# BerserkerMother/Video-Summarization

Measured on AMD Instinct MI355X. Metric: frames/sec scored (whole node), synthetic [B,T=1024,D=1024], higher is better.
Workload: dtype f32; 1 GPU; configs[2]: B=64 videos x T=1024 frames x D=1024 per GPU, scorer cfg M-A (heads 4, d_model 256, layers 4), logits + hidden state; global_batch=64, parallelism=videos sharded over 1 GPU(s), no all_gather of scores

## Files before the change

### video-summarization_amd/csrc/vs_attention.hip

```cpp
#include "vs_device.h"
#include "vs_kernels.h"

namespace {

template <int DH, int NKB, bool VARLEN = false>
__global__ __launch_bounds__(256, 2) void attn_fwd(
    const float *__restrict__ Q, const float *__restrict__ Kg, const float *__restrict__ Vg,
    const uint8_t *__restrict__ mask, float *__restrict__ out, int H, int T, float scale_log2e, int BH,
    const int *__restrict__ cu = nullptr, const int2 *__restrict__ work = nullptr, int Mtot = 0) {
    constexpr int KT = 32 * NKB, LD = DH + 4, NJ = DH / 8, ND = DH / 32;
    constexpr int F4 = KT * DH / 4 / 256;
    __shared__ __attribute__((aligned(16))) float Ks[KT * LD];
    __shared__ __attribute__((aligned(16))) float Vs[KT * LD];
    __shared__ float mb[KT];

    const int tid = threadIdx.x, lane = tid & 63, wave = tid >> 6;
    const int r = lane & 31, h = lane >> 5;
    int b, head, qt;
    size_t base, orow0;
    if constexpr (VARLEN) {
        const int2 wk = work[blockIdx.x];
        b = wk.x; qt = wk.y; head = blockIdx.y;
        const int c0 = cu[b];
        T = cu[b + 1] - c0;
// ... 744 lines not shown
    };
    if constexpr (DMA) {
#pragma unroll
        for (int u = 0; u < KAHEAD; ++u) dma_issue(u, u, true, u < VAHEAD);
#pragma unroll
        for (int u = 0; u < KAHEAD; ++u) { gload_m(u); stage_m(u % NMB); }
        gload_m(KAHEAD);
        asm volatile("s_waitcnt vmcnt(0)" ::: "memory");
    } else {
#pragma unroll
        for (int u = 0; u < KAHEAD; ++u) {
            gload_k(u); gload_m(u);
            if (u < VAHEAD) gload_v(u);
#pragma unroll
            for (int i = 0; i < KPT; ++i) stage_k1(i, u % NBUF);
            if (u < VAHEAD) {
#pragma unroll
                for (int e = 0; e < 4; ++e) stage_v1(e, u % NBUF);
            }
            stage_m(u % NMB);
        }
        gload_k(KAHEAD); gload_m(KAHEAD); gload_v(VAHEAD);
    }
    __syncthreads();
    f32x16 sa[2], sb[2];
#pragma unroll
    for (int n = 0; n < 2; ++n)
#pragma unroll
        for (int t = 0; t < 16; ++t) { sa[n][t] = 0.f; sb[n][t] = 0.f; }
#pragma unroll
    for (int ks = 0; ks < NS; ++ks)
#pragma unroll
        for (int n = 0; n < 2; ++n) {
            u32x4 ka[NP];
            k_frag(0, ks, n, ka);
            static_for<NPROD>([&](auto prc) { mma_prod(prc, ka, qreg[ks], sa[n]); });
        }

    constexpr float CMARGIN = PREC == 2 ? -8.0f : 6.0f;
    (void)CMARGIN;
    u32x4 pf[2][2][NP];
    f16x2 pmaxh = {(_Float16)0.f, (_Float16)0.f};
    float cb_a = 0.f, cb_b = 0.f;
    auto rebase = [&](f32x16 (&sv)[2], float &cb, bool raise) __attribute__((always_inline)) {
        float mx = __builtin_fmaxf(__builtin_fmaxf(sv[0][0], sv[0][1]), sv[1][0]);
        mx = __builtin_fmaxf(mx, sv[1][1]);
#pragma unroll
        for (int t = 2; t < 16; t += 2) {
            mx = __builtin_fmaxf(__builtin_fmaxf(mx, sv[0][t]), sv[0][t + 1]);
            mx = __builtin_fmaxf(__builtin_fmaxf(mx, sv[1][t]), sv[1][t + 1]);
        }
        const float raw = pair_max(mx) + cb;
        float c_new = m_run;
        if ((raise || m_run == NEG_INF) && raw + CMARGIN > m_run) {
            const float cl = __builtin_fminf(__builtin_fmaxf(raw + CMARGIN, -32768.f), 32768.f);
            const unsigned b = __builtin_bit_cast(unsigned, cl);
            constexpr unsigned LOW = PREC == 2 ? 0x1FFFu : 0xFFFFu;
            c_new = __builtin_bit_cast(float, (cl >= 0.f ? b + LOW : b) & ~LOW);
            if (PREC == 1 && __builtin_fabsf(cl) >= 8192.f) c_new = __builtin_bit_cast(float, (b + 0x8000u) & ~LOW);
            if (PREC == 2 && __builtin_fabsf(c_new) < 0.0001220703125f) c_new = cl > 0.f ? 0.0001220703125f : 0.f;
        }
        const float u_new = (c_new == NEG_INF) ? 0.f : c_new;
        const float shift = cb - u_new;
        const float alpha = __builtin_amdgcn_exp2f(m_run - u_new);
#pragma unroll
        for (int n = 0; n < 2; ++n)
#pragma unroll
            for (int t = 0; t < 16; ++t) sv[n][t] += shift;
#pragma unroll
        for (int d = 0; d <= ND; ++d)
#pragma unroll
            for (int t = 0; t < 16; ++t) o[d][t] *= alpha;
        m_run = c_new;
        cb = u_new;
        unsigned pl[NP];
        pack(-u_new, 0.f, pl);
        nbias = h == 0 ? pl[0] : 0u;
    };
    auto p_pair = [&](auto kc, f32x16 (&sv)[2]) __attribute__((always_inline)) {
        constexpr int k = decltype(kc)::value, n = k / 8, ks = (k / 4) % 2, j = k % 4;
        unsigned pl[NP];
        pack(__builtin_amdgcn_exp2f(sv[n][8 * ks + 2 * j]), __builtin_amdgcn_exp2f(sv[n][8 * ks + 2 * j + 1]), pl);
#pragma unroll
        for (int p = 0; p < NP; ++p) pf[n][ks][p][j] = pl[p];
        if constexpr (PREC == 2) pmaxh = __builtin_elementwise_max(pmaxh, __builtin_bit_cast(f16x2, pl[0]));
    };
    float sm_mx = 0.f;
    f32x2 sm_mm = {0.f, 0.f};
    auto sm_unit_max = [&](auto uc, f32x16 (&sv)[2]) __attribute__((always_inline)) {
        constexpr int U = decltype(uc)::value;
        constexpr float THR = 8.0f;
        if constexpr (U == 0) {
            sm_mx = __builtin_fmaxf(__builtin_fmaxf(sv[0][0], sv[0][1]), sv[1][0]);
            sm_mx = __builtin_fmaxf(sm_mx, sv[1][1]);
        }
        if constexpr (U < 4) {
            constexpr int t0 = U == 0 ? 2 : 4 * U;
#pragma unroll
            for (int t = t0; t < 4 * U + 4; t += 2) {
                sm_mx = __builtin_fmaxf(__builtin_fmaxf(sm_mx, sv[0][t]), sv[0][t + 1]);
                sm_mx = __builtin_fmaxf(__builtin_fmaxf(sm_mx, sv[1][t]), sv[1][t + 1]);
            }
        }
        if constexpr (U == 4) {
            const float mx = pair_max(sm_mx);
            const bool raise = mx > m_run + THR || (m_run == NEG_INF && mx != NEG_INF);
            if (__builtin_expect(__any(raise), 0)) {
                const float m_new = raise ? mx : m_run;
                const float u_new = (m_new == NEG_INF) ? 0.f : m_new;
                const float alpha = __builtin_amdgcn_exp2f(m_run - u_new);
#pragma unroll
                for (int d = 0; d <= ND; ++d)
#pragma unroll
                    for (int t = 0; t < 16; ++t) o[d][t] *= alpha;
                m_run = m_new;
            }
            const float m_use = (m_run == NEG_INF) ? 0.f : m_run;
            sm_mm[0] = m_use; sm_mm[1] = m_use;
        }
        if constexpr (U >= 5 && U < 21) {
            constexpr int k = U - 5, n = k / 8, ks = (k / 4) % 2, j = k % 4;
            const f32x2 sx = {sv[n][8 * ks + 2 * j], sv[n][8 * ks + 2 * j + 1]};
            const f32x2 dv = sx - sm_mm;
            unsigned pl[NP];
            pack(__builtin_amdgcn_exp2f(dv[0]), __builtin_amdgcn_exp2f(dv[1]), pl);
#pragma unroll
            for (int p = 0; p < NP; ++p) pf[n][ks][p][j] = pl[p];
        }
    };
    auto sm_unit = [&](auto uc, f32x16 (&sv)[2], float &cb) __attribute__((always_inline)) {
        constexpr int U = decltype(uc)::value;
        if constexpr (!FOLD) { sm_unit_max(uc, sv); return; }
        if constexpr (U == 0) {
            const float u_run = (m_run == NEG_INF) ? 0.f : m_run;
            if (__builtin_expect(__any(cb != u_run || m_run == NEG_INF), 0)) rebase(sv, cb, false);
        }
        if constexpr (U >= 1 && U < 17) p_pair(std::integral_constant<int, U - 1>{}, sv);
        if constexpr (U == 17) {
            unsigned acc = 0u;
            bool hit;
            if constexpr (PREC == 2) {
                acc = __builtin_bit_cast(unsigned, pmaxh);
                hit = (acc & 0xFFFFu) >= 0x7800u || (acc >> 16) >= 0x7800u;
                pmaxh = f16x2{(_Float16)0.f, (_Float16)0.f};
            } else {
#pragma unroll
                for (int n = 0; n < 2; ++n)
#pragma unroll
                    for (int ks = 0; ks < 2; ++ks) acc |= (pf[n][ks][0][0] | pf[n][ks][0][1]) | (pf[n][ks][0][2] | pf[n][ks][0][3]);
                hit = (acc & 0x40004000u) != 0u;
            }
            if (__builtin_expect(__any(hit), 0)) {
                const unsigned hbit = hit ? 1u : 0u;
                auto pr = __builtin_amdgcn_permlane32_swap(hbit, hbit, false, false);
                rebase(sv, cb, (((unsigned)pr[0] | (unsigned)pr[1]) & 1u) != 0u);
                static_for<16>([&](auto kc) { p_pair(kc, sv); });
                if constexpr (PREC == 2) pmaxh = f16x2{(_Float16)0.f, (_Float16)0.f};
            }
        }
    };
    constexpr int NU = FOLD ? 18 : 21;
    constexpr bool FULLPF = PREC == 1 && DH <= 64;
    constexpr int NKF = FULLPF ? NS * 2 : 2, NVF = FULLPF ? 4 * ND : 2;
    constexpr int NBIAS = FOLD ? 2 : 0;
    constexpr int NSLOT_A = 2 * NS * NPROD + NBIAS, RA = (NU + NSLOT_A - 1) / NSLOT_A;
    constexpr int NSLOT_B = 4 * (ND * NPROD + NP);
    constexpr int NITEM = KPT + 4 + 2, SB = NSLOT_B / NITEM > 0 ? NSLOT_B / NITEM : 1;

    u32x4 abl_frag = {0u, 0u, 0u, 0u};
    if constexpr ((ABL & 16) != 0) abl_frag = *(const u32x4 *)&Kb[0][0][r * LDK + 8 * h];
    auto iteration = [&](int t, f32x16 (&s_in)[2], float &cb_in, f32x16 (&s_out)[2], float &cb_out) __attribute__((always_inline)) {
        const int cur = (ABL & 4) ? 0 : t % NBUF, nxt = (ABL & 4) ? 0 : (t + 1) % NBUF;
        if (mask != nullptr || (t + 1) * KT > T) {
            const float *mp = mb[t % NMB];
#pragma unroll
            for (int n = 0; n < 2; ++n)
#pragma unroll
                for (int g = 0; g < 4; ++g) {
                    const f32x4 bv = *(const f32x4 *)&mp[32 * n + 8 * g + 4 * h];
#pragma unroll
                    for (int e = 0; e < 4; ++e) s_in[n][4 * g + e] += bv[e];
                }
        }
        cb_out = (m_run == NEG_INF) ? 0.f : m_run;
        const u32x4 nb = {nbias, 0u, 0u, 0u};
        const f32x16 zero16 = {0.f, 0.f, 0.f, 0.f, 0.f, 0.f, 0.f, 0.f, 0.f, 0.f, 0.f, 0.f, 0.f, 0.f, 0.f, 0.f};
        u32x4 ka[NKF][NP], va[NVF][NP];
        if constexpr ((ABL & 16) != 0) {
#pragma unroll
            for (int g = 0; g < NKF; ++g)
#pragma unroll
                for (int p = 0; p < NP; ++p) ka[g][p] = abl_frag;
#pragma unroll
            for (int g = 0; g < NVF; ++g)
#pragma unroll
                for (int p = 0; p < NP; ++p) va[g][p] = abl_frag;
        } else
        if constexpr (FULLPF) {
#pragma unroll
            for (int g = 0; g < NS * 2; ++g) k_frag(nxt, g % NS, g / NS, ka[g]);
        } else {
            k_frag(nxt, 0, 0, ka[0]);
        }
        __builtin_amdgcn_sched_barrier(0);
        static_for<NSLOT_A>([&](auto ic) {
            constexpr int i = decltype(ic)::value, PERN = NS * NPROD, n = i < NBIAS ? i : (i - NBIAS) / PERN,
                          w = i < NBIAS ? 0 : 1 + (i - NBIAS) % PERN;
            if constexpr (w == 0) {
                s_out[n] = mma(ones_u, nb, zero16);
            } else {
                constexpr int ks = (w - 1) / NPROD, pr = (w - 1) % NPROD, g = n * NS + ks;
                if constexpr (!FOLD && w == 1) s_out[n] = zero16;
                if constexpr (!(ABL & 16) && !FULLPF && pr == 0 && g + 1 < NS * 2) k_frag(nxt, (g + 1) % NS, (g + 1) / NS, ka[(g + 1) & 1]);
                mma_prod(std::integral_constant<int, pr>{}, ka[FULLPF ? g : (g & 1)], qreg[ks], s_out[n]);
            }
            if constexpr (!(ABL & 16) && FULLPF && i >= NBIAS && i - NBIAS < NVF) {
                constexpr int f = i - NBIAS;
                v_frag(cur, f / ND / 2, (f / ND) % 2, f % ND, va[f]);
            }
            static_for<RA>([&](auto rc) {
                constexpr int U = i * RA + decltype(rc)::value;
                if constexpr (U < NU && !(ABL & 8)) sm_unit(std::integral_constant<int, U>{}, s_in, cb_in);
            });
            __builtin_amdgcn_sched_barrier(0);
        });
        lap(1);
        if constexpr (DMA) asm volatile("s_waitcnt vmcnt(0)" ::: "memory");
        if constexpr (STAG && !(ABL & 2)) { __syncthreads(); lap(3); }
        if constexpr (!FULLPF && !(ABL & 16)) v_frag(cur, 0, 0, 0, va[0]);
        __builtin_amdgcn_sched_barrier(0);
        static_for<NSLOT_B>([&](auto ic) {
            constexpr int i = decltype(ic)::value;
            constexpr int PER = ND * NPROD + NP;
            constexpr int g = i / PER, w = i % PER, n = g / 2, ks = g % 2;
            if constexpr (w < ND * NPROD) {
                constexpr int d = w / NPROD, pr = w % NPROD, f = g * ND + d;
                if constexpr (!(ABL & 16) && !FULLPF && pr == 0 && f + 1 < 4 * ND)
                    v_frag(cur, (f + 1) / ND / 2, ((f + 1) / ND) % 2, (f + 1) % ND, va[(f + 1) & 1]);
                mma_prod(std::integral_constant<int, pr>{}, va[FULLPF ? f : (f & 1)], pf[n][ks], o[d]);
            } else {
                constexpr int p = NP - 1 - (w - ND * NPROD);
                o[ND] = mma(ones_u, pf[n][ks][p], o[ND]);
            }
            if constexpr (DMA) {
                if constexpr (!(ABL & 1) && i == 0) dma_issue(t + KAHEAD, t + VAHEAD, true, true);
                if constexpr (!(ABL & 1) && i == 4) { stage_m((t + KAHEAD) % NMB); gload_m(t + KAHEAD + 1); }
            } else
            if constexpr (!(ABL & 1) && i % SB == SB - 1 && i / SB < NITEM) {
                constexpr int item = i / SB;
                if constexpr (item < KPT) stage_k1(item, (t + KAHEAD) % NBUF);
                else if constexpr (item < KPT + 4) stage_v1(item - KPT, (t + VAHEAD) % NBUF);
                else if constexpr (item == KPT + 4) { stage_m((t + KAHEAD) % NMB); }
                else { gload_k(t + KAHEAD + 1); gload_m(t + KAHEAD + 1); gload_v(t + VAHEAD + 1); }
            }
            __builtin_amdgcn_sched_barrier(0);
        });
        lap(2);
        if constexpr (!(ABL & 2)) __syncthreads();
        lap(3);
    };

    lap(0);
    const bool late = STAG && __builtin_amdgcn_readfirstlane(wave) >= NW / 2;
    if (late) __syncthreads();
    int t = 0;
    for (; t + 1 < ntiles; t += 2) {
        iteration(t, sa, cb_a, sb, cb_b);
        iteration(t + 1, sb, cb_b, sa, cb_a);
    }
    if (t < ntiles) iteration(t, sa, cb_a, sb, cb_b);
    if (STAG && !late) __syncthreads();

    const int q = q0 + r;
    if (q < T) {
        const float inv = 1.0f / o[ND][0];
        float *op = out + (orow0 + q) * (H * DH) + head * DH;
        h16 *op16 = (h16 *)out + (orow0 + q) * (H * DH) + head * DH;
#pragma unroll
        for (int d = 0; d < ND; ++d)
#pragma unroll
            for (int g = 0; g < 4; ++g) {
                f32x4 v;
#pragma unroll
                for (int e = 0; e < 4; ++e) v[e] = o[d][4 * g + e] * inv;
                if constexpr (IO16) {
                    u32x2 u; u[0] = pack_bf16(v[0], v[1]); u[1] = pack_bf16(v[2], v[3]);
                    *(u32x2 *)(op16 + 32 * d + 8 * g + 4 * h) = u;
                } else
                *(f32x4 *)(op + 32 * d + 8 * g + 4 * h) = v;
            }
    }
    if constexpr (DIAG != 0) {
        asm volatile("s_waitcnt vmcnt(0)" ::: "memory");
        lap(7);
        dg[8] = tl - tbeg; dg[10] = __builtin_amdgcn_s_memrealtime(); dg[11] = (unsigned long long)ntiles;
        if (diag != nullptr && lane == 0) {
            unsigned long long *o_ = diag + ((size_t)blockIdx.x * NW + wave) * 16;
#pragma unroll
            for (int i = 0; i < 12; ++i) o_[i] = dg[i];
        }
    }
}

template <int DH, bool HAS_MASK, int NW, bool VARLEN = false, int DIAG = 0>
__global__ __launch_bounds__(64 * NW, 2) void attn_fwd_pipe(
    const float *__restrict__ Q, const float *__restrict__ Kg, const float *__restrict__ Vg,
    const uint8_t *__restrict__ mask, float *__restrict__ out, int H, int T, float scale_log2e, int BH,
    const int *__restrict__ cu = nullptr, const int2 *__restrict__ work = nullptr, int Mtot = 0,
    unsigned long long *__restrict__ diag = nullptr) {
    unsigned long long dg[13] = {0ull, 0ull, 0ull, 0ull, 0ull, 0ull, 0ull, 0ull, 0ull, 0ull, 0ull, 0ull, 0ull}, tbeg = 0, tl = 0;
    if constexpr (DIAG != 0) { dg[9] = __builtin_amdgcn_s_memrealtime(); tbeg = vs_stamp(); tl = tbeg; }
    auto lap = [&](int slot) __attribute__((always_inline)) {
        if constexpr (DIAG != 0) { const unsigned long long t = vs_stamp(); dg[slot] += t - tl; tl = t; }
    };
    constexpr int KT = 64, LD = DH + 4, NJ = DH / 8, ND = DH / 32;
    constexpr int NT = 64 * NW;
    constexpr int F4 = KT * DH / 4 / NT;
    constexpr int TILE = KT * LD;
    constexpr float THR = 8.0f;
    __shared__ __attribute__((aligned(16))) float smem[4 * TILE + 2 * KT];
    float *mbs = smem + 4 * TILE;

    const int tid = threadIdx.x, lane = tid & 63, wave = tid >> 6;
    const int r = lane & 31, h = lane >> 5;
    int b, head, qt;
    size_t base, orow0;
    if constexpr (VARLEN) {
        const int2 wk = work[blockIdx.x];
        b = wk.x; qt = wk.y; head = blockIdx.y;
        const int c0 = cu[b];
        T = cu[b + 1] - c0;
        base = ((size_t)head * Mtot + c0) * DH;
        orow0 = (size_t)c0;
    } else {
        int bh;
        if (!attn_block_map((T + 32 * NW - 1) / (32 * NW), BH, bh, qt)) return;
        b = bh / H; head = bh - b * H;
        base = (size_t)bh * T * DH;
        orow0 = (size_t)b * T;
    }
    const int q0 = qt * (32 * NW) + 32 * wave;
    const float NEG_INF = -__builtin_inff();
    const int ntiles = (T + KT - 1) / KT;

    float qreg[4 * NJ];
    static_assert(4 * TILE >= NW * 32 * LD || NW == 8, "LDS corner per wave");
    float *wtp = smem + wave * (32 * LD);
    {
#pragma unroll
        for (int i = 0; i < DH / 8; ++i) {
            const int idx = lane + 64 * i;
            const int row = idx / (DH / 4), c4 = (idx % (DH / 4)) * 4;
            int qr = q0 + row; qr = qr < T ? qr : T - 1;
            *(f32x4 *)&wtp[row * LD + c4] = *(const f32x4 *)(Q + base + (size_t)qr * DH + c4);
        }
#pragma unroll
        for (int j = 0; j < NJ; ++j) {
            const f32x4 v = *(const f32x4 *)&wtp[r * LD + 8 * j + 4 * h];
#pragma unroll
            for (int s = 0; s < 4; ++s) qreg[4 * j + s] = v[s] * scale_log2e;
        }
    }
    lap(12);
    __syncthreads();
    f32x16 o[ND];
#pragma unroll
    for (int d = 0; d < ND; ++d)
#pragma unroll
        for (int t = 0; t < 16; ++t) o[d][t] = 0.f;
    float m_run = NEG_INF, l_run = 0.f;
    const float ones_a = h == 0 ? 1.0f : 0.0f;

    const __amdgpu_buffer_rsrc_t krs = __builtin_amdgcn_make_buffer_rsrc(
        const_cast<float *>(Kg + base), 0, T * DH * 4, 0x00020000);
    const __amdgpu_buffer_rsrc_t vrs = __builtin_amdgcn_make_buffer_rsrc(
        const_cast<float *>(Vg + base), 0, T * DH * 4, 0x00020000);
    int voff[F4];
#pragma unroll
    for (int i = 0; i < F4; ++i) {
        const int idx = tid + NT * i;
        voff[i] = ((idx / (DH / 4)) * DH + (idx % (DH / 4)) * 4) * 4;
    }
    f32x4 pk[F4], pv[F4];
    float pm = 0.f;
    auto gload_k = [&](int i, int tile) __attribute__((always_inline)) { pk[i] = __builtin_bit_cast(f32x4, __builtin_amdgcn_raw_buffer_load_b128(krs, voff[i], tile * (KT * DH * 4), 0)); };
    auto gload_v = [&](int i, int tile) __attribute__((always_inline)) { pv[i] = __builtin_bit_cast(f32x4, __builtin_amdgcn_raw_buffer_load_b128(vrs, voff[i], tile * (KT * DH * 4), 0)); };
    auto gload_m = [&](int tile) __attribute__((always_inline)) {
        const int key = tile * KT + (tid & (KT - 1));
        float pmv = key >= T ? NEG_INF : 0.f;
        if (HAS_MASK) pmv = mask[(size_t)b * T + (key < T ? key : T - 1)] != 0 ? NEG_INF : pmv;
        pm = pmv;
    };
    auto stage_k = [&](int i, int buf) __attribute__((always_inline)) {
        const int idx = tid + NT * i;
        *(f32x4 *)&smem[buf * 2 * TILE + (idx / (DH / 4)) * LD + (idx % (DH / 4)) * 4] = pk[i];
    };
    auto stage_v = [&](int i, int buf) __attribute__((always_inline)) {
        const int idx = tid + NT * i;
        *(f32x4 *)&smem[buf * 2 * TILE + TILE + (idx / (DH / 4)) * LD + (idx % (DH / 4)) * 4] = pv[i];
    };

    float sm_mx = 0.f, sm_psum = 0.f;
    float vreg[16 * ND];
    auto fixup = [&](f32x16 &sv, float m_bias, float raw_max) __attribute__((always_inline)) {
        const float m_new = (raw_max > m_run + THR || m_run == NEG_INF) ? fmaxf(m_run, raw_max) : m_run;
        const float u_new = (m_new == NEG_INF) ? 0.f : m_new;
        const float shift = m_bias - u_new;
        const float alpha = __builtin_amdgcn_exp2f(m_run - u_new);
#pragma unroll
        for (int t = 0; t < 16; ++t) sv[t] += shift;
#pragma unroll
        for (int d = 0; d < ND; ++d)
#pragma unroll
            for (int t = 0; t < 16; ++t) o[d][t] *= alpha;
        l_run *= alpha;
        m_run = m_new;
    };
    auto sm_unit = [&](auto uc, f32x16 &sv, float m_bias, const float *mb, auto masked_tag) __attribute__((always_inline)) {
        constexpr int U = decltype(uc)::value;
        constexpr bool MASKED = decltype(masked_tag)::value;
        if constexpr (MASKED && U < 4) {
            const f32x4 bv = *(const f32x4 *)(mb + 8 * U + 4 * h);
#pragma unroll
            for (int e = 0; e < 4; ++e) sv[4 * U + e] += bv[e];
        }
        if constexpr (U == 4) {
            sm_mx = fmaxf(fmaxf(sv[0], sv[1]), sv[2]);
#pragma unroll
            for (int t = 3; t < 15; t += 2) sm_mx = fmaxf(fmaxf(sm_mx, sv[t]), sv[t + 1]);
            sm_mx = fmaxf(sm_mx, sv[15]);
        }
        if constexpr (U == 5) {
            const float raw_max = pair_max(sm_mx) + m_bias;
            const float u_run = (m_run == NEG_INF) ? 0.f : m_run;
            const bool fix = (m_bias != u_run) || (raw_max > m_run + THR) || (m_run == NEG_INF && raw_max != NEG_INF);
            if (__builtin_expect(__any(fix), 0)) fixup(sv, m_bias, raw_max);
            sm_psum = 0.f;
        }
        if constexpr (U >= 8 && U < 16) {
            constexpr int k = U - 8;
#pragma unroll
            for (int e = 0; e < 2; ++e) {
                const float pe_ = __builtin_amdgcn_exp2f(sv[2 * k + e]);
                sv[2 * k + e] = pe_;
                sm_psum += pe_;
            }
        }
        if constexpr (U == 16) l_run += pair_sum(sm_psum);
    };
    auto half_step = [&](const float *Ksrc, int blk, f32x16 &s_out, float m_bias_out, f32x16 &s_in, float m_bias_in,
                         const float *mb, const float *Vsrc, int vblk, auto masked_tag, auto stage_tag, int nbuf, int ntile) __attribute__((always_inline)) {
        constexpr bool STAGE = decltype(stage_tag)::value;
        constexpr int NSLOT = 4 * NJ, R = 32 / NSLOT;
        static_assert(NSLOT == 16 * ND, "one V operand per MFMA slot");
        const float *kp = Ksrc + (32 * blk + r) * LD + 4 * h;
        const float *vp = Vsrc + (32 * vblk + 4 * h) * LD + r;
        f32x4 ka[2];
        ka[0] = *(const f32x4 *)kp;
        const f32x16 zero = {0.f, 0.f, 0.f, 0.f, 0.f, 0.f, 0.f, 0.f, 0.f, 0.f, 0.f, 0.f, 0.f, 0.f, 0.f, 0.f};
        s_out = MFMA32(ones_a, -m_bias_out, zero);
        __builtin_amdgcn_sched_barrier(0);
        static_for<NSLOT>([&](auto ic) {
            constexpr int i = decltype(ic)::value, j = i / 4, st = i % 4;
            if constexpr (st == 0 && j + 1 < NJ) ka[(j + 1) & 1] = *(const f32x4 *)(kp + 8 * (j + 1));
            s_out = MFMA32(ka[j & 1][st], qreg[4 * j + st], s_out);
            {
                constexpr int t = i / ND, d = i % ND;
                vreg[i] = vp[((t & 3) + 8 * (t >> 2)) * LD + 32 * d];
            }
            static_for<R>([&](auto rc) {
                constexpr int U = i * R + decltype(rc)::value;
                sm_unit(std::integral_constant<int, U>{}, s_in, m_bias_in, mb, masked_tag);
                if constexpr (STAGE) {
                    if constexpr (U < 2 * F4) { if constexpr (U % 2 == 0) stage_k(U / 2, nbuf); else stage_v(U / 2, nbuf); }
                    if constexpr (U == 2 * F4) mbs[nbuf * KT + (tid & (KT - 1))] = pm;
                    if constexpr (U >= 17 && U < 17 + 2 * F4) { if constexpr ((U - 17) % 2 == 0) gload_k((U - 17) / 2, ntile); else gload_v((U - 17) / 2, ntile); }
                    if constexpr (U == 17 + 2 * F4) gload_m(ntile);
                }
            });
            __builtin_amdgcn_sched_barrier(0);
        });
    };
    auto softmax_only = [&](f32x16 &sv, float m_bias, const float *mb, const float *Vsrc, int vblk, auto masked_tag) __attribute__((always_inline)) {
        const float *vp = Vsrc + (32 * vblk + 4 * h) * LD + r;
#pragma unroll
        for (int i = 0; i < 16 * ND; ++i) vreg[i] = vp[(((i / ND) & 3) + 8 * ((i / ND) >> 2)) * LD + 32 * (i % ND)];
        static_for<32>([&](auto uc) { sm_unit(uc, sv, m_bias, mb, masked_tag); });
    };
    auto pv_acc = [&](const f32x16 &p) __attribute__((always_inline)) {
#pragma unroll
        for (int t = 0; t < 16; ++t)
#pragma unroll
            for (int d = 0; d < ND; ++d) o[d] = MFMA32(vreg[ND * t + d], p[t], o[d]);
    };

#pragma unroll
    for (int i = 0; i < F4; ++i) { gload_k(i, 0); gload_v(i, 0); }
    gload_m(0);
#pragma unroll
    for (int i = 0; i < F4; ++i) { stage_k(i, 0); stage_v(i, 0); }
    mbs[tid & (KT - 1)] = pm;
    {
        const int t1 = ntiles > 1 ? 1 : 0;
#pragma unroll
        for (int i = 0; i < F4; ++i) { gload_k(i, t1); gload_v(i, t1); }
        gload_m(t1);
    }
    __syncthreads();
    f32x16 s_cur, s_nxt;
    float mb_cur = 0.f, mb_nxt = 0.f;
    {
        const float *kp = smem + r * LD + 4 * h;
#pragma unroll
        for (int t = 0; t < 16; ++t) s_cur[t] = 0.f;
#pragma unroll
        for (int j = 0; j < NJ; ++j) {
            const f32x4 ka = *(const f32x4 *)(kp + 8 * j);
#pragma unroll
            for (int st = 0; st < 4; ++st) s_cur = MFMA32(ka[st], qreg[4 * j + st], s_cur);
        }
    }

    auto tile_step = [&](int t, auto masked_tag, auto last_tag) __attribute__((always_inline)) {
        constexpr bool LAST = decltype(last_tag)::value;
        const int buf = t & 1;
        const float *Ks = smem + buf * 2 * TILE, *Vs = Ks + TILE;
        const float *Kn = smem + (buf ^ 1) * 2 * TILE;
        __syncthreads();
        lap(1);
        mb_nxt = (m_run == NEG_INF) ? 0.f : m_run;
        half_step(Ks, 1, s_nxt, mb_nxt, s_cur, mb_cur, mbs + buf * KT, Vs, 0, masked_tag, std::integral_constant<bool, !LAST>{},
                  buf ^ 1, t + 2 < ntiles ? t + 2 : ntiles - 1);
        lap(2);
        pv_acc(s_cur);
        lap(3);
        __syncthreads();
        lap(4);
        if constexpr (!LAST) {
            mb_cur = (m_run == NEG_INF) ? 0.f : m_run;
            half_step(Kn, 0, s_cur, mb_cur, s_nxt, mb_nxt, mbs + buf * KT + 32, Vs, 1, masked_tag, std::false_type{}, 0, 0);
        } else {
            softmax_only(s_nxt, mb_nxt, mbs + buf * KT + 32, Vs, 1, masked_tag);
        }
        lap(5);
        pv_acc(s_nxt);
        lap(6);
    };
    lap(0);
    for (int t = 0; t + 1 < ntiles; ++t) tile_step(t, std::integral_constant<bool, HAS_MASK>{}, std::false_type{});
    if (HAS_MASK || (T % KT) != 0) tile_step(ntiles - 1, std::true_type{}, std::true_type{});
    else                           tile_step(ntiles - 1, std::false_type{}, std::true_type{});

    __syncthreads();
    {
        const float inv = 1.0f / l_run;
#pragma unroll
        for (int d = 0; d < ND; ++d)
#pragma unroll
            for (int g = 0; g < 4; ++g) {
                f32x4 v;
#pragma unroll
                for (int e = 0; e < 4; ++e) v[e] = o[d][4 * g + e] * inv;
                *(f32x4 *)&wtp[r * LD + 32 * d + 8 * g + 4 * h] = v;
            }
        constexpr int LPR = DH / 4, RPI = 64 / LPR;
        const int orow = lane / LPR, oc4 = (lane % LPR) * 4;
#pragma unroll
        for (int p = 0; p < 32 / RPI; ++p) {
            const int rr = orow + RPI * p, q = q0 + rr;
            const f32x4 v = *(const f32x4 *)&wtp[rr * LD + oc4];
            if (q < T) *(f32x4 *)(out + (orow0 + q) * (H * DH) + head * DH + oc4) = v;
        }
    }
    if constexpr (DIAG != 0) {
        asm volatile("s_waitcnt vmcnt(0)" ::: "memory");
        lap(7);
        dg[8] = tl - tbeg; dg[10] = __builtin_amdgcn_s_memrealtime(); dg[11] = (unsigned long long)ntiles;
        dg[0] -= dg[12];
        if (diag != nullptr && lane == 0) {
            unsigned long long *o = diag + ((size_t)blockIdx.x * NW + wave) * 16;
#pragma unroll
            for (int i = 0; i < 13; ++i) o[i] = dg[i];
        }
    }
}

}

#ifdef VS_WITH_DIAG
int vsk_diag_attention(const float *q, const float *k, const float *v, float *out, int B, int H, int T, float scale,
                       unsigned long long *diag, hipStream_t st) {
    const int BH = B * H, nq = (T + 255) / 256;
    dim3 g(8 * ((BH + 7) / 8) * nq);
    hipLaunchKernelGGL((attn_fwd_pipe<64, false, 8, false, 1>), g, dim3(512), 0, st, q, k, v, nullptr, out, H, T,
                       scale * 1.4426950408889634f, BH, nullptr, nullptr, 0, diag);
    VSK_CHECK_LAUNCH();
    return (int)g.x;
}
int vsk_diag_attention_lp(const float *q, const float *k, const float *v, float *out, int B, int H, int T, float scale,
                          int prec, unsigned long long *diag, hipStream_t st) {
    const int BH = B * H, nq = (T + 255) / 256;
    dim3 g(8 * ((BH + 7) / 8) * nq);
    const float sl2 = scale * 1.4426950408889634f;
    if (prec >= 100) {
#define VSK_ABL(A_) case A_: hipLaunchKernelGGL((attn_fwd_lp_pipe<64, 8, 1, false, true, 0, A_>), g, dim3(512), 0, st, q, k, v, nullptr, out, H, T, sl2, BH, nullptr, nullptr, 0, nullptr); break;
        switch (prec - 100) {
            VSK_ABL(0) VSK_ABL(1) VSK_ABL(2) VSK_ABL(3) VSK_ABL(4) VSK_ABL(5) VSK_ABL(7) VSK_ABL(16) VSK_ABL(17) VSK_ABL(19)
            default: return -1;
        }
#undef VSK_ABL
        VSK_CHECK_LAUNCH();
        return (int)g.x;
    }
    if (prec == 1)
        hipLaunchKernelGGL((attn_fwd_lp_pipe<64, 8, 1, false, true, 1>), g, dim3(512), 0, st, q, k, v, nullptr, out, H, T, sl2, BH,
                           nullptr, nullptr, 0, diag);
    else
        hipLaunchKernelGGL((attn_fwd_lp_pipe<64, 8, 2, false, false, 1>), g, dim3(512), 0, st, q, k, v, nullptr, out, H, T, sl2, BH,
                           nullptr, nullptr, 0, diag);
    VSK_CHECK_LAUNCH();
    return (int)g.x;
}
#endif

float vsk_attention_qscale(float scale) { return scale * 1.4426950408889634f; }

int vsk_attention(const float *q, const float *k, const float *v, const uint8_t *mask, float *out,
                  int B, int H, int T, int dh, float scale, hipStream_t st) {
    const float sl2 = vsk_attention_qscale(scale);
    const int BH = B * H;
    dim3 grid(8 * ((BH + 7) / 8) * ((T + 127) / 128));
#ifdef VS_WITH_DIAG
    const bool legacy = vsk_options().attn_legacy != 0;
    if (dh == 32 && legacy)
        hipLaunchKernelGGL((attn_fwd<32, 2>), grid, dim3(256), 0, st, q, k, v, mask, out, H, T, sl2, BH);
    else if (dh == 64 && legacy)
        hipLaunchKernelGGL((attn_fwd<64, 2>), grid, dim3(256), 0, st, q, k, v, mask, out, H, T, sl2, BH);
    else
#endif
    if (dh == 32 || dh == 64) {
        const int r8 = (T + 255) / 256 * 256, r4 = (T + 127) / 128 * 128;
        const bool wide = !vsk_options().attn_nw4 && r8 * 100 <= r4 * 105;
        const int nq = wide ? r8 / 256 : r4 / 128;
        dim3 g(8 * ((BH + 7) / 8) * nq), blk(wide ? 512 : 256);
#define VSK_ATTN(DH_, MASK_, NW_) \
    hipLaunchKernelGGL((attn_fwd_pipe<DH_, MASK_, NW_, false>), g, blk, 0, st, q, k, v, mask, out, H, T, sl2, BH, nullptr, nullptr, 0, nullptr)
        if (dh == 32) {
            if (mask) { if (wide) VSK_ATTN(32, true, 8); else VSK_ATTN(32, true, 4); }
            else      { if (wide) VSK_ATTN(32, false, 8); else VSK_ATTN(32, false, 4); }
        } else {
            if (mask) { if (wide) VSK_ATTN(64, true, 8); else VSK_ATTN(64, true, 4); }
            else      { if (wide) VSK_ATTN(64, false, 8); else VSK_ATTN(64, false, 4); }
        }
#undef VSK_ATTN
    }
    else if (dh == 128)
        hipLaunchKernelGGL((attn_fwd<128, 1>), grid, dim3(256), 0, st, q, k, v, mask, out, H, T, sl2, BH);
    else
        return -1;
    VSK_CHECK_LAUNCH();
    return 0;
}

int vsk_attention_splitkv(const float *q, const float *k, const float *v, const uint8_t *mask, float *out,
                          int B, int H, int T, int dh, float scale, hipStream_t st) {
    const float sl2 = vsk_attention_qscale(scale);
    const dim3 grid(((T + 31) / 32) * B * H);
    if (dh == 64) hipLaunchKernelGGL((attn_fwd_splitkv<64>), grid, dim3(512), 0, st, q, k, v, mask, out, H, T, sl2, B * H);
    else if (dh == 128) hipLaunchKernelGGL((attn_fwd_splitkv<128>), grid, dim3(512), 0, st, q, k, v, mask, out, H, T, sl2, B * H);
    else if (dh == 32) hipLaunchKernelGGL((attn_fwd_splitkv<32>), grid, dim3(512), 0, st, q, k, v, mask, out, H, T, sl2, B * H);
    else return -1;
    VSK_CHECK_LAUNCH();
    return 0;
}

int vsk_attention_packed(const float *q, const float *k, const float *v, float *out, int H, int Mtot, int dh,
                         float scale, const int *cu, const int *work, int nwork, int nw, int prec, hipStream_t st) {
    const float sl2 = vsk_attention_qscale(scale);
    if (nwork <= 0) return 0;
    if (prec == (1 | VSK_STORE16) && dh == 64 && nw == 8 && vsk_options().attn_w64)
        return vsk_attention_bf16_w64_packed(q, k, v, out, H, Mtot, cu, work, nwork, st);
    dim3 grid(nwork, H);
    const int2 *wk = (const int2 *)work;
#define VSK_ATTN_PX(DH_, NW_) \
    hipLaunchKernelGGL((attn_fwd_pipe<DH_, false, NW_, true>), grid, dim3(64 * NW_), 0, st, q, k, v, nullptr, out, H, 0, sl2, 0, cu, wk, Mtot, nullptr)
#define VSK_ATTN_PE(DH_, NW_, P_) \
    hipLaunchKernelGGL((attn_fwd_lp_pipe<DH_, NW_, P_, true>), grid, dim3(64 * NW_), 0, st, q, k, v, nullptr, out, H, 0, sl2, 0, cu, wk, Mtot)
#define VSK_ATTN_P16(DH_, NW_) \
    hipLaunchKernelGGL((attn_fwd_lp_pipe<DH_, NW_, 1, true, true>), grid, dim3(64 * NW_), 0, st, q, k, v, nullptr, out, H, 0, sl2, 0, cu, wk, Mtot)
    if (prec == (1 | VSK_STORE16)) {
        if (dh == 64 && nw == 8) VSK_ATTN_P16(64, 8);
        else if (dh == 64 && nw == 4) VSK_ATTN_P16(64, 4);
        else if (dh == 32 && nw == 4) VSK_ATTN_P16(32, 4);
        else return -1;
    } else if (prec == 2) {
        if (dh == 64 && nw == 8) VSK_ATTN_PE(64, 8, 2);
        else if (dh == 64 && nw == 4) VSK_ATTN_PE(64, 4, 2);
        else if (dh == 32 && nw == 4) VSK_ATTN_PE(32, 4, 2);
        else return -1;
    } else if (prec == 1) {
        if (dh == 128 && nw == 8) VSK_ATTN_PE(128, 8, 1);
        else if (dh == 64 && nw == 8) VSK_ATTN_PE(64, 8, 1);
        else if (dh == 64 && nw == 4) VSK_ATTN_PE(64, 4, 1);
        else if (dh == 32 && nw == 4) VSK_ATTN_PE(32, 4, 1);
        else return -1;
    } else {
        if (dh == 128 && nw == 4)
            hipLaunchKernelGGL((attn_fwd<128, 1, true>), grid, dim3(256), 0, st, q, k, v, nullptr, out, H, 0, sl2, 0, cu, wk, Mtot);
        else if (dh == 64 && nw == 8) VSK_ATTN_PX(64, 8);
        else if (dh == 64 && nw == 4) VSK_ATTN_PX(64, 4);
        else if (dh == 32 && nw == 8) VSK_ATTN_PX(32, 8);
        else if (dh == 32 && nw == 4) VSK_ATTN_PX(32, 4);
        else return -1;
    }
#undef VSK_ATTN_PX
#undef VSK_ATTN_PE
#undef VSK_ATTN_P16
    VSK_CHECK_LAUNCH();
    return 0;
}

int vsk_attention_bf16(const float *q, const float *k, const float *v, const uint8_t *mask, float *out,
                       int B, int H, int T, int dh, float scale, int prec, hipStream_t st) {
    const float sl2 = vsk_attention_qscale(scale);
    const int BH = B * H;
    const int r8 = (T + 255) / 256 * 256, r4 = (T + 127) / 128 * 128;
    const bool wide = dh == 64 && !vsk_options().attn_nw4 && r8 * 100 <= r4 * 105;
    dim3 grid(8 * ((BH + 7) / 8) * (wide ? r8 / 256 : r4 / 128));
    const bool simple = vsk_options().attn_lp_simple != 0;
    if (dh == 128) {
        if (prec != 1 && prec != (1 | VSK_STORE16)) return -1;
        dim3 g128(8 * ((BH + 7) / 8) * (r8 / 256));
        if (prec == (1 | VSK_STORE16))
            hipLaunchKernelGGL((attn_fwd_lp_pipe<128, 8, 1, false, true>), g128, dim3(512), 0, st, q, k, v, mask, out, H, T, sl2, BH);
        else
        hipLaunchKernelGGL((attn_fwd_lp_pipe<128, 8, 1>), g128, dim3(512), 0, st, q, k, v, mask, out, H, T, sl2, BH);
        VSK_CHECK_LAUNCH();
        return 0;
    }
#define VSK_ATTN_LP(KERN_, P_)                                                                                           \
    if (dh == 64 && wide)                                                                                                \
        hipLaunchKernelGGL((KERN_<64, 8, P_>), grid, dim3(512), 0, st, q, k, v, mask, out, H, T, sl2, BH);               \
    else if (dh == 64)                                                                                                   \
        hipLaunchKernelGGL((KERN_<64, 4, P_>), grid, dim3(256), 0, st, q, k, v, mask, out, H, T, sl2, BH);               \
    else if (dh == 32)                                                                                                   \
        hipLaunchKernelGGL((KERN_<32, 4, P_>), grid, dim3(256), 0, st, q, k, v, mask, out, H, T, sl2, BH);               \
    else                                                                                                                 \
        return -1;
    if (prec == (1 | VSK_STORE16)) {
        if (dh == 64 && wide && vsk_options().attn_w64) {
            const int rc = vsk_attention_bf16_w64(q, k, v, mask, out, B, H, T, st);
            if (rc != -1) return rc;
        }
        if (dh == 64 && wide)
            hipLaunchKernelGGL((attn_fwd_lp_pipe<64, 8, 1, false, true>), grid, dim3(512), 0, st, q, k, v, mask, out, H, T, sl2, BH);
        else if (dh == 64)
            hipLaunchKernelGGL((attn_fwd_lp_pipe<64, 4, 1, false, true>), grid, dim3(256), 0, st, q, k, v, mask, out, H, T, sl2, BH);
        else if (dh == 32)
            hipLaunchKernelGGL((attn_fwd_lp_pipe<32, 4, 1, false, true>), grid, dim3(256), 0, st, q, k, v, mask, out, H, T, sl2, BH);
        else
            return -1;
    } else
    if (simple) { if (prec == 2) { VSK_ATTN_LP(attn_fwd_lp, 2) } else { VSK_ATTN_LP(attn_fwd_lp, 1) } }
    else        { if (prec == 2) { VSK_ATTN_LP(attn_fwd_lp_pipe, 2) } else { VSK_ATTN_LP(attn_fwd_lp_pipe, 1) } }
#undef VSK_ATTN_LP
    VSK_CHECK_LAUNCH();
    return 0;
}
```

Baseline: 11.97 million frames/s.

## Streamline pipelined attention inner loop: cached bias, max3 reductions, unrolled buffers

Result: faster. 12.12 million frames/s (median of 6 runs) (+1.3%).

```diff
diff --git a/video-summarization_amd/csrc/vs_attention.hip b/video-summarization_amd/csrc/vs_attention.hip
--- a/video-summarization_amd/csrc/vs_attention.hip
+++ b/video-summarization_amd/csrc/vs_attention.hip
@@ -1070,6 +1070,27 @@
     }
 }
 
+__device__ __forceinline__ float max3f(float a, float b, float c) {
+    float d;
+    asm("v_max3_f32 %0, %1, %2, %3" : "=v"(d) : "v"(a), "v"(b), "v"(c));
+    return d;
+}
+__device__ __forceinline__ float max2f(float a, float b) {
+    float d;
+    asm("v_max_f32 %0, %1, %2" : "=v"(d) : "v"(a), "v"(b));
+    return d;
+}
+__device__ __forceinline__ float pair_max2f(float x) {
+    const unsigned u = __builtin_bit_cast(unsigned, x);
+    auto pr = __builtin_amdgcn_permlane32_swap(u, u, false, false);
+    return max2f(__builtin_bit_cast(float, (unsigned)pr[0]), __builtin_bit_cast(float, (unsigned)pr[1]));
+}
+__device__ __forceinline__ f32x16 mfma32_keep_c(float a, float b, const f32x16 &c) {
+    f32x16 d;
+    asm("v_mfma_f32_32x32x2_f32 %0, %1, %2, %3" : "=&v"(d) : "v"(a), "v"(b), "v"(c));
+    return d;
+}
+
 template <int DH, bool HAS_MASK, int NW, bool VARLEN = false, int DIAG = 0>
 __global__ __launch_bounds__(64 * NW, 2) void attn_fwd_pipe(
     const float *__restrict__ Q, const float *__restrict__ Kg, const float *__restrict__ Vg,
@@ -1136,8 +1157,10 @@
     for (int d = 0; d < ND; ++d)
 #pragma unroll
         for (int t = 0; t < 16; ++t) o[d][t] = 0.f;
-    float m_run = NEG_INF, l_run = 0.f;
-    const float ones_a = h == 0 ? 1.0f : 0.0f;
+    float m_run = NEG_INF, l_run = 0.f, u_run = 0.f, thr_run = NEG_INF;
+    f32x16 cbias;
+#pragma unroll
+    for (int t = 0; t < 16; ++t) cbias[t] = 0.f;
 
     const __amdgpu_buffer_rsrc_t krs = __builtin_amdgcn_make_buffer_rsrc(
         const_cast<float *>(Kg + base), 0, T * DH * 4, 0x00020000);
@@ -1154,19 +1177,16 @@
     auto gload_k = [&](int i, int tile) __attribute__((always_inline)) { pk[i] = __builtin_bit_cast(f32x4, __builtin_amdgcn_raw_buffer_load_b128(krs, voff[i], tile * (KT * DH * 4), 0)); };
     auto gload_v = [&](int i, int tile) __attribute__((always_inline)) { pv[i] = __builtin_bit_cast(f32x4, __builtin_amdgcn_raw_buffer_load_b128(vrs, voff[i], tile * (KT * DH * 4), 0)); };
     auto gload_m = [&](int tile) __attribute__((always_inline)) {
-        const int key = tile * KT + (tid & (KT - 1));
+        const int key = (HAS_MASK ? tile : ntiles - 1) * KT + (tid & (KT - 1));
         float pmv = key >= T ? NEG_INF : 0.f;
         if (HAS_MASK) pmv = mask[(size_t)b * T + (key < T ? key : T - 1)] != 0 ? NEG_INF : pmv;
         pm = pmv;
     };
-    auto stage_k = [&](int i, int buf) __attribute__((always_inline)) {
-        const int idx = tid + NT * i;
-        *(f32x4 *)&smem[buf * 2 * TILE + (idx / (DH / 4)) * LD + (idx % (DH / 4)) * 4] = pk[i];
-    };
-    auto stage_v = [&](int i, int buf) __attribute__((always_inline)) {
-        const int idx = tid + NT * i;
-        *(f32x4 *)&smem[buf * 2 * TILE + TILE + (idx / (DH / 4)) * LD + (idx % (DH / 4)) * 4] = pv[i];
-    };
+    static_assert(NT % (DH / 4) == 0, "a staging pass covers whole key rows");
+    constexpr int SROW = (NT / (DH / 4)) * LD;
+    float *const sdst = smem + (tid / (DH / 4)) * LD + (tid % (DH / 4)) * 4;
+    auto stage_k = [&](int i, int buf) __attribute__((always_inline)) { *(f32x4 *)&sdst[buf * 2 * TILE + i * SROW] = pk[i]; };
+    auto stage_v = [&](int i, int buf) __attribute__((always_inline)) { *(f32x4 *)&sdst[buf * 2 * TILE + TILE + i * SROW] = pv[i]; };
 
     float sm_mx = 0.f, sm_psum = 0.f;
     float vreg[16 * ND];
@@ -1182,7 +1202,10 @@
 #pragma unroll
             for (int t = 0; t < 16; ++t) o[d][t] *= alpha;
         l_run *= alpha;
-        m_run = m_new;
+        m_run = m_new; u_run = u_new; thr_run = m_new + THR;
+        const float nb = 0.0f - u_new;
+#pragma unroll
+        for (int t = 0; t < 16; ++t) cbias[t] = nb;
     };
     auto sm_unit = [&](auto uc, f32x16 &sv, float m_bias, const float *mb, auto masked_tag) __attribute__((always_inline)) {
         constexpr int U = decltype(uc)::value;
@@ -1193,17 +1216,14 @@
             for (int e = 0; e < 4; ++e) sv[4 * U + e] += bv[e];
         }
         if constexpr (U == 4) {
-            sm_mx = fmaxf(fmaxf(sv[0], sv[1]), sv[2]);
-#pragma unroll
-            for (int t = 3; t < 15; t += 2) sm_mx = fmaxf(fmaxf(sm_mx, sv[t]), sv[t + 1]);
-            sm_mx = fmaxf(sm_mx, sv[15]);
+            const float a0 = max3f(sv[0], sv[1], sv[2]), a1 = max3f(sv[3], sv[4], sv[5]), a2 = max3f(sv[6], sv[7], sv[8]);
+            const float a3 = max3f(sv[9], sv[10], sv[11]), a4 = max3f(sv[12], sv[13], sv[14]);
+            sm_mx = max2f(max3f(a0, a1, a2), max3f(a3, a4, sv[15]));
         }
         if constexpr (U == 5) {
-            const float raw_max = pair_max(sm_mx) + m_bias;
-            const float u_run = (m_run == NEG_INF) ? 0.f : m_run;
-            const bool fix = (m_bias != u_run) || (raw_max > m_run + THR) || (m_run == NEG_INF && raw_max != NEG_INF);
+            const float raw_max = pair_max2f(sm_mx) + m_bias;
+            const bool fix = (m_bias != u_run) || (raw_max > thr_run);
             if (__builtin_expect(__any(fix), 0)) fixup(sv, m_bias, raw_max);
-            sm_psum = 0.f;
         }
         if constexpr (U >= 8 && U < 16) {
             constexpr int k = U - 8;
@@ -1211,27 +1231,28 @@
             for (int e = 0; e < 2; ++e) {
                 const float pe_ = __builtin_amdgcn_exp2f(sv[2 * k + e]);
                 sv[2 * k + e] = pe_;
-                sm_psum += pe_;
+                if (k == 0 && e == 0) sm_psum = pe_; else sm_psum += pe_;
             }
         }
         if constexpr (U == 16) l_run += pair_sum(sm_psum);
     };
-    auto half_step = [&](const float *Ksrc, int blk, f32x16 &s_out, float m_bias_out, f32x16 &s_in, float m_bias_in,
+    const float *const kfrag = smem + r * LD + 4 * h;
+    const float *const vfrag = smem + 4 * h * LD + r;
+    auto half_step = [&](const float *Ksrc, int blk, f32x16 &s_out, f32x16 &s_in, float m_bias_in,
                          const float *mb, const float *Vsrc, int vblk, auto masked_tag, auto stage_tag, int nbuf, int ntile) __attribute__((always_inline)) {
         constexpr bool STAGE = decltype(stage_tag)::value;
         constexpr int NSLOT = 4 * NJ, R = 32 / NSLOT;
         static_assert(NSLOT == 16 * ND, "one V operand per MFMA slot");
-        const float *kp = Ksrc + (32 * blk + r) * LD + 4 * h;
-        const float *vp = Vsrc + (32 * vblk + 4 * h) * LD + r;
+        const float *kp = kfrag + ((Ksrc - smem) + 32 * blk * LD);
+        const float *vp = vfrag + ((Vsrc - smem) + 32 * vblk * LD);
         f32x4 ka[2];
         ka[0] = *(const f32x4 *)kp;
-        const f32x16 zero = {0.f, 0.f, 0.f, 0.f, 0.f, 0.f, 0.f, 0.f, 0.f, 0.f, 0.f, 0.f, 0.f, 0.f, 0.f, 0.f};
-        s_out = MFMA32(ones_a, -m_bias_out, zero);
-        __builtin_amdgcn_sched_barrier(0);
+        const f32x16 c0 = cbias;
         static_for<NSLOT>([&](auto ic) {
             constexpr int i = decltype(ic)::value, j = i / 4, st = i % 4;
             if constexpr (st == 0 && j + 1 < NJ) ka[(j + 1) & 1] = *(const f32x4 *)(kp + 8 * (j + 1));
-            s_out = MFMA32(ka[j & 1][st], qreg[4 * j + st], s_out);
+            if constexpr (i == 0) s_out = mfma32_keep_c(ka[0][0], qreg[0], c0);
+            else s_out = MFMA32(ka[j & 1][st], qreg[4 * j + st], s_out);
             {
                 constexpr int t = i / ND, d = i % ND;
                 vreg[i] = vp[((t & 3) + 8 * (t >> 2)) * LD + 32 * d];
@@ -1246,11 +1267,13 @@
                     if constexpr (U == 17 + 2 * F4) gload_m(ntile);
                 }
             });
+            if constexpr (i == 1) asm volatile("" :: "v"(c0));
             __builtin_amdgcn_sched_barrier(0);
         });
     };
     auto softmax_only = [&](f32x16 &sv, float m_bias, const float *mb, const float *Vsrc, int vblk, auto masked_tag) __attribute__((always_inline)) {
-        const float *vp = Vsrc + (32 * vblk + 4 * h) * LD + r;
+        const float *vp = vfrag + ((Vsrc - smem) + 32 * vblk * LD);
+        __builtin_amdgcn_sched_barrier(0);
 #pragma unroll
         for (int i = 0; i < 16 * ND; ++i) vreg[i] = vp[(((i / ND) & 3) + 8 * ((i / ND) >> 2)) * LD + 32 * (i % ND)];
         static_for<32>([&](auto uc) { sm_unit(uc, sv, m_bias, mb, masked_tag); });
@@ -1289,15 +1312,15 @@
         }
     }
 
-    auto tile_step = [&](int t, auto masked_tag, auto last_tag) __attribute__((always_inline)) {
+    auto tile_step = [&](int t, auto buf_tag, auto masked_tag, auto last_tag) __attribute__((always_inline)) {
         constexpr bool LAST = decltype(last_tag)::value;
-        const int buf = t & 1;
+        const int buf = buf_tag;
         const float *Ks = smem + buf * 2 * TILE, *Vs = Ks + TILE;
         const float *Kn = smem + (buf ^ 1) * 2 * TILE;
         __syncthreads();
         lap(1);
-        mb_nxt = (m_run == NEG_INF) ? 0.f : m_run;
-        half_step(Ks, 1, s_nxt, mb_nxt, s_cur, mb_cur, mbs + buf * KT, Vs, 0, masked_tag, std::integral_constant<bool, !LAST>{},
+        mb_nxt = u_run;
+        half_step(Ks, 1, s_nxt, s_cur, mb_cur, mbs + buf * KT, Vs, 0, masked_tag, std::integral_constant<bool, !LAST>{},
                   buf ^ 1, t + 2 < ntiles ? t + 2 : ntiles - 1);
         lap(2);
         pv_acc(s_cur);
@@ -1305,8 +1328,8 @@
         __syncthreads();
         lap(4);
         if constexpr (!LAST) {
-            mb_cur = (m_run == NEG_INF) ? 0.f : m_run;
-            half_step(Kn, 0, s_cur, mb_cur, s_nxt, mb_nxt, mbs + buf * KT + 32, Vs, 1, masked_tag, std::false_type{}, 0, 0);
+            mb_cur = u_run;
+            half_step(Kn, 0, s_cur, s_nxt, mb_nxt, mbs + buf * KT + 32, Vs, 1, masked_tag, std::false_type{}, 0, 0);
         } else {
             softmax_only(s_nxt, mb_nxt, mbs + buf * KT + 32, Vs, 1, masked_tag);
         }
@@ -1315,9 +1338,29 @@
         lap(6);
     };
     lap(0);
-    for (int t = 0; t + 1 < ntiles; ++t) tile_step(t, std::integral_constant<bool, HAS_MASK>{}, std::false_type{});
-    if (HAS_MASK || (T % KT) != 0) tile_step(ntiles - 1, std::true_type{}, std::true_type{});
-    else                           tile_step(ntiles - 1, std::false_type{}, std::true_type{});
+    constexpr std::integral_constant<int, 0> B0{};
+    constexpr std::integral_constant<int, 1> B1{};
+    constexpr std::integral_constant<bool, HAS_MASK> MK{};
+    const bool dead_keys = HAS_MASK || (T % KT) != 0;
+    int t = 0;
+    if constexpr (NW != 8) {
+        for (; t + 1 < ntiles; ++t) tile_step(t, t & 1, MK, std::false_type{});
+        if (dead_keys) tile_step(t, t & 1, std::true_type{}, std::true_type{});
+        else           tile_step(t, t & 1, std::false_type{}, std::true_type{});
+    } else {
+        for (; t + 2 < ntiles; t += 2) {
+            tile_step(t, B0, MK, std::false_type{});
+            tile_step(t + 1, B1, MK, std::false_type{});
+        }
+        if (t + 2 == ntiles) {
+            tile_step(t, B0, MK, std::false_type{});
+            if (dead_keys) tile_step(t + 1, B1, std::true_type{}, std::true_type{});
+            else           tile_step(t + 1, B1, std::false_type{}, std::true_type{});
+        } else {
+            if (dead_keys) tile_step(t, B0, std::true_type{}, std::true_type{});
+            else           tile_step(t, B0, std::false_type{}, std::true_type{});
+        }
+    }
 
     __syncthreads();
     {
```
